# anerisheth19/CNN-MobileNet-V1-implementation-on-AWS-FPGA-using-OpenCL

Hardware: AMD Instinct MI355X
Metric: images/sec MobileNet-V1 1.0x224 fp32, batch 256; per-stage HBM GB/s vs roofline (higher is better)
Workload: dtype f32

## Files before the change

cnn-mobilenet-v1-implementation-on-aws-fpga-using-opencl_amd/csrc/mbn_abi.hip:

```cpp
#include "mbn_internal.h"

#include <initializer_list>
#include <new>

mbn_tunables g_mbn_tune;

namespace {

struct Span { const void *p; double bytes; const char *what; };

int span_check(mbn_context *ctx, const Span *sp, int n)
{
    std::lock_guard<std::mutex> lk(ctx->mu);
    if (ctx->allocs.empty()) return MBN_OK;
    for (int i = 0; i < n; i++) {
        if (!sp[i].p || sp[i].bytes <= 0) continue;
        const uintptr_t a = (uintptr_t)sp[i].p;
        auto it = ctx->allocs.upper_bound(a);
        if (it == ctx->allocs.begin()) continue;
        --it;
        if (a >= it->first + it->second) continue;
        const double room = (double)(it->first + it->second - a);
        if (sp[i].bytes > room) {
            snprintf(ctx->last_error, sizeof(ctx->last_error), "%s: call touches %.0f bytes, %.0f left in its %zu-byte mbn_alloc buffer",
// ... 729 lines not shown
                int channels, int classes, void *workspace, size_t workspace_bytes, void *stream)
{
    if (!ctx || !logits || !in || !fc_w || !workspace || batch <= 0 || rows <= 0 || cols <= 0 || channels <= 0 || classes <= 0) return MBN_EINVAL;
    if (batch > 4 || channels < 64 || channels > 1024 || (channels % 64) != 0) return MBN_EUNSUPPORTED;
    if (workspace_bytes < mbn_pool_fc_ws_bytes(channels, classes)) return MBN_EINVAL;
    hipStream_t s = stream ? (hipStream_t)stream : ctx->stream;
    MBN_SPANS(ctx, { in, 4.0 * batch * rows * cols * channels, "pool_fc input" }, { logits, 4.0 * batch * classes, "pool_fc logits" },
              { fc_w, 4.0 * classes * channels, "pool_fc filter" }, { workspace, (double)mbn_pool_fc_ws_bytes(channels, classes), "pool_fc workspace" });
    Scope sc(ctx, s);
    return sc.finish(mbn_launch_f32_pool_fc(ctx, s, (float *)logits, (const float *)in, (const float *)fc_w, (const float *)fc_bias, workspace,
                                            batch, rows * cols, channels, classes, 0, nullptr, nullptr, nullptr));
}

int mbn_classifier_tail_fused(mbn_context *ctx, void *topk_idx_i32, void *topk_prob_f32, void *probs, void *logits, const void *in, const void *fc_w,
                              const void *fc_bias, int batch, int rows, int cols, int channels, int classes, int k, void *workspace,
                              size_t workspace_bytes, void *stream)
{
    if (!ctx || !topk_idx_i32 || !topk_prob_f32 || !logits || !in || !fc_w || !workspace || batch <= 0 || rows <= 0 || cols <= 0 || channels <= 0 ||
        classes <= 0 || k < 1 || k > 8)
        return MBN_EINVAL;
    if (batch > 4 || channels < 64 || channels > 1024 || (channels % 64) != 0 || classes > 1024) return MBN_EUNSUPPORTED;
    if (workspace_bytes < mbn_pool_fc_ws_bytes(channels, classes)) return MBN_EINVAL;
    hipStream_t s = stream ? (hipStream_t)stream : ctx->stream;
    MBN_SPANS(ctx, { in, 4.0 * batch * rows * cols * channels, "classifier_tail_fused input" }, { logits, 4.0 * batch * classes, "classifier_tail_fused logits" },
              { fc_w, 4.0 * classes * channels, "classifier_tail_fused filter" }, { workspace, (double)mbn_pool_fc_ws_bytes(channels, classes), "classifier_tail_fused workspace" },
              { probs, 4.0 * batch * classes, "classifier_tail_fused probs" }, { topk_idx_i32, 4.0 * batch * k, "classifier_tail_fused idx" },
              { topk_prob_f32, 4.0 * batch * k, "classifier_tail_fused prob" });
    Scope sc(ctx, s);
    return sc.finish(mbn_launch_f32_pool_fc(ctx, s, (float *)logits, (const float *)in, (const float *)fc_w, (const float *)fc_bias, workspace,
                                            batch, rows * cols, channels, classes, k, (float *)probs, (int32_t *)topk_idx_i32, (float *)topk_prob_f32));
}

static int stem_fused_impl(mbn_context *ctx, void *out, const void *image, const void *w1, const void *s1, const void *b1,
                           const void *wd, const void *s2, const void *b2, const void *wp, const void *s3, const void *b3,
                           int batch, int res, int c1, int c3, void *stream, int in_u8, int bf16)
{
    if (!ctx || !out || !image) return MBN_EINVAL;
    hipStream_t s = stream ? (hipStream_t)stream : ctx->stream;
    if (mbn_stem_envelope(batch, res, c1, c3) != MBN_OK) return MBN_EUNSUPPORTED;
    MBN_SPANS(ctx, { image, (in_u8 ? 1.0 : 4.0) * batch * res * res * 3, "stem image" },
              { out, (bf16 ? 2.0 : 4.0) * batch * (res / 2) * (res / 2) * c3, "stem output" });
    if (check_ptrs({ w1, s1, b1, wd, s2, b2, wp, s3, b3 }) != MBN_OK) return MBN_EUNSUPPORTED;
    if (((uintptr_t)out % 16) != 0 || ((uintptr_t)image % (in_u8 ? 2 : 8)) != 0) return MBN_EINVAL;
    Scope sc(ctx, s);
    return sc.finish(mbn_launch_f32_stem(ctx, s, (float *)out, (const float *)image, (const float *)w1, (const float *)s1,
                                         (const float *)b1, (const float *)wd, (const float *)s2, (const float *)b2,
                                         (const float *)wp, (const float *)s3, (const float *)b3, batch, res, c1, c3, in_u8, bf16));
}

int mbn_stem_fused(mbn_context *ctx, void *out, const void *image, const void *w1, const void *s1, const void *b1,
                   const void *wd, const void *s2, const void *b2, const void *wp, const void *s3, const void *b3,
                   int batch, int res, int c1, int c3, void *stream)
{
    return stem_fused_impl(ctx, out, image, w1, s1, b1, wd, s2, b2, wp, s3, b3, batch, res, c1, c3, stream, 0, 0);
}

int mbn_stem_fused_u8(mbn_context *ctx, void *out, const void *image_u8, const void *w1, const void *s1, const void *b1,
                      const void *wd, const void *s2, const void *b2, const void *wp, const void *s3, const void *b3,
                      int batch, int res, int c1, int c3, void *stream)
{
    return stem_fused_impl(ctx, out, image_u8, w1, s1, b1, wd, s2, b2, wp, s3, b3, batch, res, c1, c3, stream, 1, 0);
}

int mbn_stem_fused_ex(mbn_context *ctx, void *out, const void *image, const void *w1, const void *s1, const void *b1,
                      const void *wd, const void *s2, const void *b2, const void *wp, const void *s3, const void *b3,
                      int batch, int res, int c1, int c3, int flags, void *stream)
{
    if (flags & ~(MBN_STEM_IN_U8 | MBN_STEM_BF16)) return MBN_EINVAL;
    return stem_fused_impl(ctx, out, image, w1, s1, b1, wd, s2, b2, wp, s3, b3, batch, res, c1, c3, stream,
                           (flags & MBN_STEM_IN_U8) != 0, (flags & MBN_STEM_BF16) != 0);
}

int mbn_dwpw_fused(mbn_context *ctx, void *out, const void *in, const void *wd, const void *s2, const void *b2,
                   const void *wp, const void *s3, const void *b3, int batch, int in_rows, int in_cols, int out_rows,
                   int out_cols, int cin, int cout, int stride, int pad_top, int pad_left, void *stream)
{
    if (!ctx) return MBN_EINVAL;
    hipStream_t s = stream ? (hipStream_t)stream : ctx->stream;
    const mbn_block_shape sh = { batch, in_rows, in_cols, out_rows, out_cols, cin, cout, stride, pad_top, pad_left };
    const mbn_block_params p = { wd, s2, b2, wp, s3, b3 };
    int rc = check_ptrs({ in, wd, s2, b2, wp, s3, b3, out });
    if (rc == MBN_OK) rc = mbn_block_envelope(&sh, MBN_DT_F32);
    if (rc != MBN_OK) return rc;
    MBN_SPANS(ctx, { in, 4.0 * batch * in_rows * in_cols * cin, "dwpw input" },
              { out, 4.0 * batch * out_rows * out_cols * cout, "dwpw output" }, { wd, 36.0 * cin, "dwpw depthwise filter" },
              { wp, 4.0 * cin * cout, "dwpw pointwise filter" });
    Scope sc(ctx, s);
    if (g_mbn_tune.pw_emul != 0 && g_mbn_tune.dwpw_variant == 0 && mbn_launch_f32_dwpw2_x6(ctx, s, sh, out, in, p) == MBN_OK)
        return sc.finish(MBN_OK);
    const int dv = g_mbn_tune.dwpw_variant;
    if ((dv == 11 || dv >= 300 || (dv == 0 && MBN_DWPW3_DEFAULT(stride, cin))) && mbn_f32_dwpw3_eligible(ctx, sh))
        return sc.finish(mbn_launch_f32_dwpw3(ctx, s, sh, out, in, p));
    const long tiles256 = (((long)batch * out_rows * out_cols + 127) / 128) * (cout / 256);
    const bool small = tiles256 < ctx->num_cus;
    if (dv != 1 && (dv >= 2 || (cout % 256) != 0 || small || stride == 2))
        return sc.finish(mbn_launch_f32_dwpw2(ctx, s, sh, out, in, p));
    return sc.finish(mbn_launch_f32_dwpw(ctx, s, sh, out, in, p));
}

int mbn_blocks_resident_bf16(mbn_context *ctx, void *out, const void *in, const mbn_block_params *blocks, int nblocks, int batch,
                             int rows, int cols, int channels, void *stream)
{
    if (!ctx || !out || !in || !blocks || batch <= 0) return MBN_EINVAL;
    const mbn_block_shape sh = { batch, rows, cols, rows, cols, channels, channels, 1, 1, 1 };
    if (mbn_resident_envelope(&sh, nblocks) != MBN_OK) return MBN_EUNSUPPORTED;
    hipStream_t s = stream ? (hipStream_t)stream : ctx->stream;
    const double act = 2.0 * batch * rows * cols * channels;
    MBN_SPANS(ctx, { in, act, "resident blocks input" }, { out, act, "resident blocks output" });
    for (int i = 0; i < nblocks; i++) {
        if (!blocks[i].wd || !blocks[i].s2 || !blocks[i].b2 || !blocks[i].wp_bf16 || !blocks[i].s3 || !blocks[i].b3) return MBN_EINVAL;
        MBN_SPANS(ctx, { blocks[i].wd, 36.0 * channels, "resident blocks depthwise filter" }, { blocks[i].wp_bf16, 2.0 * channels * channels, "resident blocks pointwise filter" },
                  { blocks[i].s2, 4.0 * channels, "resident blocks scale" }, { blocks[i].b3, 4.0 * channels, "resident blocks shift" });
    }
    int rc = check_ptrs({ out, in });
    for (int i = 0; i < nblocks && rc == MBN_OK; i++) rc = check_ptrs(blocks[i]);
    if (rc != MBN_OK) return rc;
    Scope sc(ctx, s);
    return sc.finish(mbn_launch_bf16_res_blocks(ctx, s, out, in, blocks, nblocks, batch, rows, cols));
}

int mbn_tail_resident_bf16(mbn_context *ctx, void *out, const void *in, const mbn_block_params *blocks, int batch, int rows, int cols, int c0, int c1,
                           void *stream)
{
    if (!ctx || !out || !in || !blocks || batch <= 0) return MBN_EINVAL;
    const mbn_block_shape b0 = { batch, rows, cols, rows / 2, cols / 2, c0, c1, 2, 0, 0 };
    const mbn_block_shape b1 = { batch, rows / 2, cols / 2, rows / 2, cols / 2, c1, c1, 1, 1, 1 };
    if (mbn_tail_envelope(&b0, &b1) != MBN_OK) return MBN_EUNSUPPORTED;
    hipStream_t s = stream ? (hipStream_t)stream : ctx->stream;
    MBN_SPANS(ctx, { in, 2.0 * batch * rows * cols * c0, "resident tail input" }, { out, 2.0 * batch * c1, "resident tail output" });
    for (int i = 0; i < 2; i++) {
        if (!blocks[i].wd || !blocks[i].s2 || !blocks[i].b2 || !blocks[i].wp_bf16 || !blocks[i].s3 || !blocks[i].b3) return MBN_EINVAL;
        const int ci = i ? c1 : c0;
        MBN_SPANS(ctx, { blocks[i].wd, 36.0 * ci, "resident tail depthwise filter" }, { blocks[i].wp_bf16, 2.0 * ci * c1, "resident tail pointwise filter" },
                  { blocks[i].s2, 4.0 * ci, "resident tail scale" }, { blocks[i].b2, 4.0 * ci, "resident tail shift" },
                  { blocks[i].s3, 4.0 * c1, "resident tail scale" }, { blocks[i].b3, 4.0 * c1, "resident tail shift" });
    }
    int rc = ((uintptr_t)out % 2) ? MBN_EUNSUPPORTED : check_ptrs({ in });
    for (int i = 0; i < 2 && rc == MBN_OK; i++) rc = check_ptrs(blocks[i]);
    if (rc != MBN_OK) return rc;
    Scope sc(ctx, s);
    return sc.finish(mbn_launch_bf16_tail(ctx, s, out, in, blocks, batch, rows, cols));
}

int mbn_dwpw_fused_bf16(mbn_context *ctx, void *out, const void *in, const void *wd, const void *s2, const void *b2,
                        const void *wp_bf16, const void *s3, const void *b3, int batch, int in_rows, int in_cols, int out_rows,
                        int out_cols, int cin, int cout, int stride, int pad_top, int pad_left, void *stream)
{
    if (!ctx) return MBN_EINVAL;
    hipStream_t s = stream ? (hipStream_t)stream : ctx->stream;
    const mbn_block_shape sh = { batch, in_rows, in_cols, out_rows, out_cols, cin, cout, stride, pad_top, pad_left };
    const mbn_block_params p = { wd, s2, b2, wp_bf16, s3, b3 };
    int rc = check_ptrs({ in, wd, s2, b2, wp_bf16, s3, b3, out });
    if (rc == MBN_OK) rc = mbn_block_envelope(&sh, MBN_DT_BF16);
    if (rc != MBN_OK) return rc;
    MBN_SPANS(ctx, { in, 2.0 * batch * in_rows * in_cols * cin, "dwpw input" },
              { out, 2.0 * batch * out_rows * out_cols * cout, "dwpw output" }, { wd, 36.0 * cin, "dwpw depthwise filter" },
              { wp_bf16, 2.0 * cin * cout, "dwpw pointwise filter" });
    Scope sc(ctx, s);
#ifdef MBN_LAB
    if (g_mbn_tune.dwpw_variant == 1 && (cout % 128) == 0 && (cin % 64) == 0)
        return sc.finish(mbn_launch_bf16_dwpw(ctx, s, sh, out, in, p));
#endif
    return sc.finish(mbn_launch_bf16_dwpw2(ctx, s, sh, out, in, p));
}

int mbn_convert_f32_to_bf16(mbn_context *ctx, void *dst_bf16, const void *src_f32, size_t count, void *stream)
{
    if (!ctx || !dst_bf16 || !src_f32) return MBN_EINVAL;
    if (count == 0) return MBN_OK;
    hipStream_t s = stream ? (hipStream_t)stream : ctx->stream;
    MBN_SPANS(ctx, { src_f32, 4.0 * count, "convert source" }, { dst_bf16, 2.0 * count, "convert destination" });
    Scope sc(ctx, s);
    return sc.finish(mbn_launch_convert(ctx, s, dst_bf16, src_f32, count, 1));
// ... 47 lines not shown
```

cnn-mobilenet-v1-implementation-on-aws-fpga-using-opencl_amd/csrc/mbn_f32_pw.hip:

```cpp
#include "mbn_internal.h"
#include "mbn_epilogue.h"

namespace {

typedef float f4 __attribute__((ext_vector_type(4)));
typedef mbn_f16v f16v;
typedef __bf16 bf8 __attribute__((ext_vector_type(8)));

#ifdef MBN_LAB
__device__ unsigned long long g_pw_clk[8][4];
#endif

__device__ unsigned long long g_pw_clk_acc[9][2];

struct PwArgs {
    void *out;
    const void *in, *filt;
    const float *scale, *shift;
    long m;
    int k, n, act;
    int mt, nt;
    int out_f32;
    int fast_epi;
    int loop2;
// ... 373 lines not shown
                }
            }
        }
        __builtin_amdgcn_sched_barrier(0);
        if (!more) break;
        vb = nvb;
    }
#ifdef MBN_LAB
    if (clk) { g_pw_clk[blockIdx.x][1] = __builtin_amdgcn_s_memtime(); g_pw_clk[blockIdx.x][3] = __builtin_amdgcn_s_memrealtime(); }
#endif
    if (hclk) {
        atomicAdd(&g_pw_clk_acc[blockIdx.x][0], __builtin_amdgcn_s_memtime() - hc0);
        atomicAdd(&g_pw_clk_acc[blockIdx.x][1], __builtin_amdgcn_s_memrealtime() - hr0);
        if (blockIdx.x == 0) atomicAdd(&g_pw_clk_acc[8][0], 1ull);
    }
}

template <typename T>
__global__ __launch_bounds__(256) void pw_generic(PwArgs a)
{
    const long t = (long)blockIdx.x * blockDim.x + threadIdx.x;
    if (t >= a.m * a.n) return;
    const long row = t / a.n;
    const int col = (int)(t % a.n);
    const T *ip = reinterpret_cast<const T *>(a.in) + row * a.k, *fp = reinterpret_cast<const T *>(a.filt) + (long)col * a.k;
    float acc = 0.f;
    for (int i = 0; i < a.k; i++) acc = fmaf((float)ip[i], (float)fp[i], acc);
    float v = fmaf(acc, a.scale ? a.scale[col] : 1.f, a.shift ? a.shift[col] : 0.f);
    if (a.act == MBN_ACT_RELU6) v = fminf(fmaxf(v, 0.f), 6.f);
    else if (a.act == MBN_ACT_RELU) v = fmaxf(v, 0.f);
    if (sizeof(T) == 4 || a.out_f32) reinterpret_cast<float *>(a.out)[t] = v;
    else reinterpret_cast<__bf16 *>(a.out)[t] = (__bf16)v;
}

template <typename T, int BM, int BN, int WM, int WN>
void launch_cfg(PwArgs &a, hipStream_t s, int num_cus)
{
    constexpr int NT = 64 * (BM / WM) * (BN / WN);
    constexpr int BKE = 8 * (16 / (int)sizeof(T));
    a.mt = (int)((a.m + BM - 1) / BM);
    a.nt = (a.n + BN - 1) / BN;
    const int nbuf = a.k <= BKE ? 1 : 2;
    const int lds_bytes = nbuf * (BM + BN) * BKB + (nbuf == 2 ? 2 * SSMAX * 4 : 0);
    int per_cu = 160 * 1024 / lds_bytes;
    const int wave_cap = 32 / (NT / 64);
    if (per_cu > wave_cap) per_cu = wave_cap;
    if (per_cu > 4) per_cu = 4;
    if (g_mbn_tune.misc > 0) per_cu = g_mbn_tune.misc;
    const long nwg = (long)a.mt * a.nt;
    long grid_l = (long)num_cus * per_cu;
    if (grid_l > nwg || g_mbn_tune.misc >= 1000 || nbuf == 1) grid_l = nwg;
    a.xn = 1;
    {
        const double filt_bytes = (double)a.n * a.k * sizeof(T);
        int xn = filt_bytes >= 16.0 * 1048576 ? 4 : filt_bytes >= 4.0 * 1048576 ? 2 : 1;
        if (g_mbn_tune.pw_xn > 0) xn = g_mbn_tune.pw_xn;
        if ((xn == 2 || xn == 4) && grid_l < nwg && (grid_l % 8) == 0 && a.nt >= xn && a.mt >= 8 / xn) a.xn = xn;
    }
    const dim3 grid((unsigned)grid_l), block(NT);
    const bool kfull = (a.k % BKE) == 0;
    const bool glds = kfull && nbuf == 2 && g_mbn_tune.pw_stage != 1;
    if (nbuf == 1) {
        if (kfull) hipLaunchKernelGGL((pw_gemm<T, BM, BN, WM, WN, 1, true, false>), grid, block, 0, s, a);
        else hipLaunchKernelGGL((pw_gemm<T, BM, BN, WM, WN, 1, false, false>), grid, block, 0, s, a);
    } else {
#ifdef MBN_LAB
        if (glds && sizeof(T) == 4 && g_mbn_tune.exp1 > 0 && ((BM == 64 && BN == 64) || (BM == 128 && BN == 128))) {
            switch (g_mbn_tune.exp1) {
#define MBN_ABL_CASE(v) case v: hipLaunchKernelGGL((pw_gemm<T, BM, BN, WM, WN, 2, true, true, v>), grid, block, 0, s, a); return;
            MBN_ABL_CASE(1) MBN_ABL_CASE(2) MBN_ABL_CASE(3) MBN_ABL_CASE(4) MBN_ABL_CASE(7) MBN_ABL_CASE(8) MBN_ABL_CASE(9) MBN_ABL_CASE(10) MBN_ABL_CASE(12) MBN_ABL_CASE(15)
#undef MBN_ABL_CASE
            default: break;
            }
        }
#endif
        if (glds) hipLaunchKernelGGL((pw_gemm<T, BM, BN, WM, WN, 2, true, true>), grid, block, 0, s, a);
#ifdef MBN_LAB
        else if (kfull) hipLaunchKernelGGL((pw_gemm<T, BM, BN, WM, WN, 2, true, false>), grid, block, 0, s, a);
#endif
        else hipLaunchKernelGGL((pw_gemm<T, BM, BN, WM, WN, 2, false, false>), grid, block, 0, s, a);
    }
}

}

int mbn_launch_f32_pointwise(const mbn_call &c, void *out, const void *in, const void *filt, long m, int cin,
                             int op_size)
{
    const bool bf = c.dtype == MBN_DT_BF16;
    PwArgs a;
    a.out = out; a.in = in; a.filt = filt; a.scale = c.scale; a.shift = c.shift;
    a.m = m; a.k = cin; a.n = op_size; a.act = c.act; a.mt = a.nt = 0;
    a.out_f32 = bf && (c.io_flags & MBN_IO_OUT_F32) ? 1 : 0;
    a.loop2 = (g_mbn_tune.conv_variant == 8 || ((cin / (bf ? 64 : 32)) & 1) || (cin % (bf ? 64 : 32)) ||
               (double)m * cin * (bf ? 2 : 4) >= 4294967296.0 || (double)op_size * cin * (bf ? 2 : 4) >= 4294967296.0) ? 0 : 1;
    a.no_ss = g_mbn_tune.conv_variant == 7 ? 1 : 0;
    a.no_cw = g_mbn_tune.exp0 == 77 ? 1 : 0;
    a.clk = g_mbn_tune.pw_clock.load(std::memory_order_relaxed) ? 1 : 0;
    a.fast_epi = (g_mbn_tune.conv_variant == 9 || (double)m * op_size * 4.0 >= 4294967296.0) ? 0 : 1;
    if (m <= 0 || (long)((m + 31) / 32) * ((op_size + 31) / 32) > 0x7fffffffL) return MBN_EINVAL;
    const int epc = bf ? 8 : 4;
    const bool fast = (cin % epc) == 0 && ((uintptr_t)in % 16) == 0 && ((uintptr_t)filt % 16) == 0;
    if (!fast) {
        long total = m * op_size;
        dim3 grid((unsigned)((total + 255) / 256));
        if (bf) hipLaunchKernelGGL(pw_generic<__bf16>, grid, dim3(256), 0, c.stream, a);
        else hipLaunchKernelGGL(pw_generic<float>, grid, dim3(256), 0, c.stream, a);
        return MBN_OK;
    }
    const int ring_mode = g_mbn_tune.pw_ring;
    if (!bf && g_mbn_tune.pw_emul != 0 && mbn_launch_f32_pw_emul(c, (float *)out, (const float *)in, (const float *)filt, m, cin, op_size) == MBN_OK)
        return MBN_OK;
    if (!bf && g_mbn_tune.pw_tile == 0 && mbn_launch_f32_pw_splitk(c, (float *)out, (const float *)in, (const float *)filt, m, cin, op_size) == MBN_OK)
        return MBN_OK;
#ifdef MBN_LAB
    if (bf && (c.io_flags & MBN_IO_FILT_PACKED) && ring_mode == 6 && g_mbn_tune.pw_tile == 0 &&
        mbn_launch_bf16_pw_wide(c, out, in, (const char *)filt + mbn_packed_filter_offset(op_size, cin), m, cin, op_size) == MBN_OK)
        return MBN_OK;
#endif
#ifdef MBN_LAB
    if (bf && ring_mode == 7 && g_mbn_tune.pw_tile == 0) {
        long done = 0;
        if (mbn_launch_bf16_pw_big(c, out, in, filt, m, cin, op_size, &done) == MBN_OK) {
            if (done < m && g_mbn_tune.exp2 < 98)
                return mbn_launch_f32_pointwise(c, (char *)out + done * op_size * 2, (const char *)in + done * cin * 2, filt, m - done, cin, op_size);
            return MBN_OK;
        }
    }
#endif
#ifdef MBN_LAB
    if (bf && ring_mode == 8 && g_mbn_tune.pw_tile == 0 && mbn_launch_bf16_pw_rf(c, out, in, filt, m, cin, op_size) == MBN_OK)
        return MBN_OK;
#endif
    if (bf && (ring_mode == 0 || ring_mode == 5 || ring_mode == 8) && cin >= 256 && g_mbn_tune.pw_tile == 0 && mbn_launch_bf16_pw_stream(c, out, in, filt, m, cin, op_size, true) == MBN_OK)
        return MBN_OK;
    if (bf && (ring_mode == 4 || ((ring_mode == 0 || ring_mode == 6) && (cin <= 128 || (cin <= 256 && op_size <= 256)))) && g_mbn_tune.pw_tile == 0 &&
        mbn_launch_bf16_pw_stream(c, out, in, filt, m, cin, op_size) == MBN_OK)
        return MBN_OK;
#ifdef MBN_LAB
    if (bf && ring_mode >= 2 && (ring_mode == 2 || cin == 64) && g_mbn_tune.pw_tile == 0 &&
        mbn_launch_bf16_pw_ring(c, out, in, filt, m, cin, op_size) == MBN_OK)
        return MBN_OK;
#endif
    if (!bf && (g_mbn_tune.pw_tile == 9 || (g_mbn_tune.pw_tile == 0 && MBN_PW3_DEFAULT(m, cin, op_size, c.ctx->num_cus))) &&
        mbn_launch_f32_pw3(c, (float *)out, (const float *)in, (const float *)filt, m, cin, op_size) == MBN_OK)
        return MBN_OK;
    int tile = g_mbn_tune.pw_tile;
    if (tile == 9 || tile == 10) tile = 0;
    if (!MBN_LAB_BUILD && tile != 2 && tile != 3 && tile != 5) tile = 0;
    if (tile == 0) {
        const long big_tiles = ((m + 127) / 128) * ((op_size + 63) / 64);
        if (big_tiles < 2L * c.ctx->num_cus || op_size <= 64 || m <= 16384) tile = 3;
        else if (!bf && (cin >= 512 || (cin >= 256 && op_size >= 512))) tile = 3;
        else if ((bf || cin <= 256) && op_size >= 128) tile = 5;
        else tile = 2;
    }
    const int cus = c.ctx->num_cus;
    if (bf) {
        switch (tile) {
        case 3:
            if (op_size >= 128) launch_cfg<__bf16, 64, 128, 32, 64>(a, c.stream, cus);
            else launch_cfg<__bf16, 64, 64, 32, 32>(a, c.stream, cus);
            break;
        case 5: launch_cfg<__bf16, 128, 128, 32, 64>(a, c.stream, cus); break;
        case 2: launch_cfg<__bf16, 128, 64, 64, 32>(a, c.stream, cus); break;
#ifdef MBN_LAB
// ... 57 lines not shown
```

cnn-mobilenet-v1-implementation-on-aws-fpga-using-opencl_amd/csrc/mbn_internal.h:

```cpp
#pragma once
#include <hip/hip_runtime.h>
#include <stdint.h>
#include <stdio.h>
#include <string.h>

#include <atomic>
#include <map>
#include <mutex>
#include <vector>

#include "mbn.h"
#include "mbn_envelope.h"

struct mbn_emul_img {
    void *p = nullptr;
    size_t bytes = 0;
    size_t src_bytes = 0;
    bool built = false;
};

struct mbn_context {
    int device = 0;
    hipStream_t stream = nullptr;
    hipEvent_t ev_start = nullptr, ev_stop = nullptr;
// ... 59 lines not shown
};
extern mbn_tunables g_mbn_tune;

struct mbn_call {
    mbn_context *ctx;
    hipStream_t stream;
    int batch;
    int act;
    int pad_top, pad_left;
    int in_rows, in_cols;
    int cin;
    int g0, g1;
    uint32_t quirks;
    const float *scale, *shift;
    int dtype;
    int io_flags;
};

int mbn_launch_lit_convolute(const mbn_call &c, uint8_t *out, const uint8_t *r, const uint8_t *g, const uint8_t *b,
                             const int32_t *filt, int rows, int cols, int fs, int stride, int op_size);
int mbn_launch_lit_depthwise(const mbn_call &c, uint8_t *out, const uint8_t *in, const int32_t *filt, int rows,
                             int cols, int fs, int stride, int op_size);
int mbn_launch_lit_pointwise(const mbn_call &c, uint8_t *out, const uint8_t *in, const int32_t *filt, int rows,
                             int cols, int cin, int op_size);
int mbn_launch_lit_pool(const mbn_call &c, uint8_t *out, const uint8_t *in, int rows, int cols, int fs, int op_size);

int mbn_launch_f32_conv(const mbn_call &c, void *out, const void *in, const float *filt, int rows, int cols, int fs,
                        int stride, int op_size);
int mbn_launch_f32_depthwise(const mbn_call &c, void *out, const void *in, const float *filt, int rows, int cols,
                             int fs, int stride, int channels);
int mbn_launch_f32_pointwise(const mbn_call &c, void *out, const void *in, const void *filt, long m, int cin,
                             int op_size);
int mbn_launch_f32_pw_splitk(const mbn_call &c, float *out, const float *in, const float *filt, long m, int cin, int op_size);
int mbn_launch_f32_pw_emul(const mbn_call &c, float *out, const float *in, const float *filt, long m, int cin, int op_size);
int mbn_pw_emul_filter_image(mbn_context *ctx, hipStream_t stream, const float *filt, int n, int k, int bn, int paired,
                             const unsigned **img, unsigned *bytes);
void mbn_pw_emul_invalidate(mbn_context *ctx, const void *dst, size_t bytes);
int mbn_launch_bf16_pw_ring(const mbn_call &c, void *out, const void *in, const void *filt, long m, int cin, int op_size);
int mbn_launch_bf16_pw_wide(const mbn_call &c, void *out, const void *in, const void *fpk, long m, int cin, int op_size);
int mbn_launch_pack_filter_bf16(mbn_context *ctx, hipStream_t s, void *dst, const void *src, int n, int k);
int mbn_bf16_pw_wide_eligible(long m, int cin, int op_size);
int mbn_launch_bf16_pw_rf(const mbn_call &c, void *out, const void *in, const void *filt, long m, int cin, int op_size);
int mbn_launch_bf16_pw_stream(const mbn_call &c, void *out, const void *in, const void *filt, long m, int cin, int op_size, bool m16 = false);
int mbn_launch_bf16_pw_big(const mbn_call &c, void *out, const void *in, const void *filt, long m, int cin, int op_size, long *rows_done);
int mbn_launch_f32_pool(const mbn_call &c, void *out, const void *in, int rows, int cols, int fs, int channels);
size_t mbn_pool_fc_ws_bytes(int channels, int classes);
int mbn_launch_f32_pool_fc(mbn_context *ctx, hipStream_t s, float *out, const float *in, const float *w, const float *bias, void *ws,
                           int batch, int pix, int channels, int classes, int k, float *probs, int32_t *topk_idx, float *topk_prob);
static inline void mbn_udiv_magic(unsigned d, unsigned *m, unsigned *s)
{
    if (d <= 1) { *m = 0; *s = 0; return; }
    unsigned l = 0;
    while ((1u << l) < d) l++;
    const unsigned long long p = 1ull << (31 + l);
    *m = (unsigned)((p + d - 1) / d);
    *s = l - 1;
}

int mbn_launch_f32_dwpw(mbn_context *ctx, hipStream_t stream, const mbn_block_shape &s, void *out, const void *in, const mbn_block_params &p);
int mbn_launch_f32_dwpw2(mbn_context *ctx, hipStream_t stream, const mbn_block_shape &s, void *out, const void *in, const mbn_block_params &p);
int mbn_launch_f32_dwpw2_x6(mbn_context *ctx, hipStream_t stream, const mbn_block_shape &s, void *out, const void *in, const mbn_block_params &p);
int mbn_launch_bf16_dwpw(mbn_context *ctx, hipStream_t stream, const mbn_block_shape &s, void *out, const void *in, const mbn_block_params &p);
int mbn_launch_bf16_dwpw2(mbn_context *ctx, hipStream_t stream, const mbn_block_shape &s, void *out, const void *in, const mbn_block_params &p);
template <typename Args>
static inline void mbn_block_args(Args &a, const mbn_block_shape &s, void *out, const void *in, const mbn_block_params &p, double esize)
{
    a.out = (decltype(a.out))out; a.in = (decltype(a.in))in;
    a.wd = (const float *)p.wd; a.s2 = (const float *)p.s2; a.b2 = (const float *)p.b2; a.s3 = (const float *)p.s3; a.b3 = (const float *)p.b3;
    a.m = (long)s.batch * s.out_rows * s.out_cols;
    a.h = s.in_rows; a.w = s.in_cols; a.ho = s.out_rows; a.wo = s.out_cols;
    a.cin = s.cin; a.cout = s.cout; a.pad_top = s.pad_top; a.pad_left = s.pad_left;
    mbn_udiv_magic((unsigned)s.out_cols, &a.wo_m, &a.wo_s);
    mbn_udiv_magic((unsigned)s.out_rows, &a.ho_m, &a.ho_s);
    a.in_bytes = (unsigned)(esize * s.batch * s.in_rows * s.in_cols * s.cin);
}
#define MBN_PW3_DEFAULT(m, cin, n, cus) ((cin) <= 256 && (n) <= 256 && (m) >= 128L * (cus))
int mbn_launch_f32_pw3(const mbn_call &c, float *out, const float *in, const float *filt, long m, int cin, int op_size);
int mbn_launch_bf16_tail(mbn_context *ctx, hipStream_t stream, void *out, const void *in, const mbn_block_params *blocks, int batch, int rows, int cols);
int mbn_launch_bf16_res_blocks(mbn_context *ctx, hipStream_t stream, void *out, const void *in, const mbn_block_params *blocks, int nblocks, int batch,
                               int rows, int cols);
#define MBN_DWPW3_DEFAULT(stride, cin) ((stride) == 1 && (cin) >= 128)
int mbn_f32_dwpw3_eligible(const mbn_context *ctx, const mbn_block_shape &s);
int mbn_launch_f32_dwpw3(mbn_context *ctx, hipStream_t stream, const mbn_block_shape &s, void *out, const void *in, const mbn_block_params &p);
int mbn_launch_f32_stem(mbn_context *ctx, hipStream_t stream, float *out, const float *in, const float *w1,
                        const float *s1, const float *b1, const float *wd, const float *s2, const float *b2,
                        const float *wp, const float *s3, const float *b3, int batch, int res, int c1, int c3, int in_u8, int bf16);
int mbn_launch_convert(mbn_context *ctx, hipStream_t s, void *dst, const void *src, size_t count, int to_bf16);
int mbn_launch_f32_softmax(mbn_context *ctx, hipStream_t s, float *probs, int32_t *argmax, const float *logits,
                           int batch, int classes);
int mbn_launch_f32_softmax_topk(mbn_context *ctx, hipStream_t s, float *probs, int32_t *topk_idx, float *topk_prob,
                                const float *logits, int batch, int classes, int k);
int mbn_launch_normalize(mbn_context *ctx, hipStream_t s, float *out, const uint8_t *in, size_t count, float scale,
                         float bias);

static inline int mbn_same_pad(int in, int out, int k, int stride)
{
    int total = (out - 1) * stride + k - in;
    if (total < 0) total = 0;
    return total / 2;
}
```

cnn-mobilenet-v1-implementation-on-aws-fpga-using-opencl_amd/host/mbn_envelope.c:

```c
#include "mbn_envelope.h"
#include "mbn.h"

int mbn_block_envelope(const mbn_block_shape *s, int dtype)
{
    const int bf = dtype == MBN_DT_BF16;
    if (!bf && dtype != MBN_DT_F32) return MBN_EUNSUPPORTED;
    if (s->batch <= 0 || (s->stride != 1 && s->stride != 2) || s->cin > MBN_CMAX || s->cout > MBN_COUT_MAX || (s->out_cols & 1) ||
        s->out_rows <= 0 || s->out_cols <= 0 || s->in_rows <= 0 || s->in_cols <= 0 || s->pad_top < 0 || s->pad_left < 0)
        return MBN_EUNSUPPORTED;
    if (bf ? (s->cin != 32 && (s->cin < 64 || (s->cin % 64) != 0)) || s->cout < 64 || (s->cout % 64) != 0
           : s->cin < 32 || (s->cin % 32) != 0 || s->cout < 128 || (s->cout % 128) != 0)
        return MBN_EUNSUPPORTED;
    const double es = bf ? 2.0 : 4.0;
    if (es * s->batch * s->in_rows * s->in_cols * s->cin >= (double)MBN_OOB) return MBN_EUNSUPPORTED;
    if ((long)s->batch * s->out_rows * s->out_cols > 0x7fffff00L) return MBN_EUNSUPPORTED;
    if (es * ((double)s->batch * s->out_rows * s->out_cols + 256.0) * s->cout >= 4294967296.0) return MBN_EUNSUPPORTED;
    return MBN_OK;
}

int mbn_resident_envelope(const mbn_block_shape *s, int nblocks)
{
    if (s->cin != 256 || s->cout != 256 || s->stride != 1 || s->pad_top != 1 || s->pad_left != 1 || s->in_rows < 1 || s->in_cols < 1 ||
        s->out_rows != s->in_rows || s->out_cols != s->in_cols || nblocks < 1 || nblocks > MBN_RES_MAXBLK)
        return MBN_EUNSUPPORTED;
    if (s->in_rows * s->in_cols > MBN_RES_YROWS || (s->in_rows + 2) * (s->in_cols + 2) > MBN_RES_XPIX) return MBN_EUNSUPPORTED;
    return MBN_OK;
}

int mbn_tail_envelope(const mbn_block_shape *b0, const mbn_block_shape *b1)
{
    const int h = b0->in_rows, w = b0->in_cols;
    if (b0->cin != 256 || b0->cout != 512 || h < 2 || w < 2 || h > MBN_TAIL_MAXSIDE || w > MBN_TAIL_MAXSIDE || (h & 1) || (w & 1))
        return MBN_EUNSUPPORTED;
    if (b0->stride != 2 || b0->pad_top != 0 || b0->pad_left != 0 || b0->out_rows != h / 2 || b0->out_cols != w / 2) return MBN_EUNSUPPORTED;
    if (b1->batch != b0->batch || b1->cin != b0->cout || b1->cout != b0->cout || b1->stride != 1 || b1->pad_top != 1 || b1->pad_left != 1 ||
        b1->in_rows != b0->out_rows || b1->in_cols != b0->out_cols || b1->out_rows != b1->in_rows || b1->out_cols != b1->in_cols)
        return MBN_EUNSUPPORTED;
    if (2.0 * b0->batch * h * w * b0->cin >= 4294967296.0) return MBN_EUNSUPPORTED;
    return MBN_OK;
}

int mbn_stem_envelope(int batch, int res, int c1, int c3)
{
    if (!((c1 == 32 && c3 == 64) || (c1 == 16 && c3 == 32)) || res < 32 || (res % 32) != 0 || batch <= 0) return MBN_EUNSUPPORTED;
    if ((long)batch * (res / 2 / MBN_STEM_TH) * (res / 2 / MBN_STEM_TW) >= 0x7fffffffL) return MBN_EUNSUPPORTED;
    return MBN_OK;
}
```

cnn-mobilenet-v1-implementation-on-aws-fpga-using-opencl_amd/host/mbn_envelope.h:

```cpp
#pragma once

#ifdef __cplusplus
extern "C" {
#endif

#define MBN_CMAX 1024
#define MBN_COUT_MAX 1024
#define MBN_OOB 0xF0000000u
#define MBN_RES_XPIX 144
#define MBN_RES_YROWS 104
#define MBN_RES_MAXBLK 8
#define MBN_TAIL_MAXSIDE 10
#define MBN_STEM_TH 8
#define MBN_STEM_TW 16

typedef struct mbn_block_shape {
    int batch, in_rows, in_cols, out_rows, out_cols, cin, cout, stride, pad_top, pad_left;
} mbn_block_shape;

int mbn_block_envelope(const mbn_block_shape *s, int dtype);
int mbn_resident_envelope(const mbn_block_shape *s, int nblocks);
int mbn_tail_envelope(const mbn_block_shape *b0, const mbn_block_shape *b1);
int mbn_stem_envelope(int batch, int res, int c1, int c3);

#ifdef __cplusplus
}
#endif
```

Before: 91970.

## Add fused depthwise-into-GEMM dwpw4 kernel for wide stride-1 f32 blocks

```diff
diff --git a/cnn-mobilenet-v1-implementation-on-aws-fpga-using-opencl_amd/csrc/mbn_abi.hip b/cnn-mobilenet-v1-implementation-on-aws-fpga-using-opencl_amd/csrc/mbn_abi.hip
--- a/cnn-mobilenet-v1-implementation-on-aws-fpga-using-opencl_amd/csrc/mbn_abi.hip
+++ b/cnn-mobilenet-v1-implementation-on-aws-fpga-using-opencl_amd/csrc/mbn_abi.hip
@@ -835,13 +835,16 @@
     int rc = check_ptrs({ in, wd, s2, b2, wp, s3, b3, out });
     if (rc == MBN_OK) rc = mbn_block_envelope(&sh, MBN_DT_F32);
     if (rc != MBN_OK) return rc;
+    const int dv = g_mbn_tune.dwpw_variant;
+    const bool gemm_form = mbn_block_gemm_envelope(&sh) == MBN_OK && g_mbn_tune.pw_emul == 0 && dv == 0;
+    if (!gemm_form && (out_cols & 1)) return MBN_EUNSUPPORTED;
     MBN_SPANS(ctx, { in, 4.0 * batch * in_rows * in_cols * cin, "dwpw input" },
               { out, 4.0 * batch * out_rows * out_cols * cout, "dwpw output" }, { wd, 36.0 * cin, "dwpw depthwise filter" },
               { wp, 4.0 * cin * cout, "dwpw pointwise filter" });
     Scope sc(ctx, s);
+    if (gemm_form) return sc.finish(mbn_launch_f32_dwpw4(ctx, s, sh, out, in, p));
     if (g_mbn_tune.pw_emul != 0 && g_mbn_tune.dwpw_variant == 0 && mbn_launch_f32_dwpw2_x6(ctx, s, sh, out, in, p) == MBN_OK)
         return sc.finish(MBN_OK);
-    const int dv = g_mbn_tune.dwpw_variant;
     if ((dv == 11 || dv >= 300 || (dv == 0 && MBN_DWPW3_DEFAULT(stride, cin))) && mbn_f32_dwpw3_eligible(ctx, sh))
         return sc.finish(mbn_launch_f32_dwpw3(ctx, s, sh, out, in, p));
     const long tiles256 = (((long)batch * out_rows * out_cols + 127) / 128) * (cout / 256);
diff --git a/cnn-mobilenet-v1-implementation-on-aws-fpga-using-opencl_amd/csrc/mbn_f32_pw.hip b/cnn-mobilenet-v1-implementation-on-aws-fpga-using-opencl_amd/csrc/mbn_f32_pw.hip
--- a/cnn-mobilenet-v1-implementation-on-aws-fpga-using-opencl_amd/csrc/mbn_f32_pw.hip
+++ b/cnn-mobilenet-v1-implementation-on-aws-fpga-using-opencl_amd/csrc/mbn_f32_pw.hip
@@ -479,6 +479,224 @@
     }
 }
 
+struct Dwpw4Args {
+    float *out;
+    const float *in, *wd, *s2, *b2, *wp, *s3, *b3;
+    long m;
+    int h, w, ho, wo, cin, cout, pad_top, pad_left;
+    unsigned in_bytes;
+    int mt, nt, xn;
+};
+
+template <int BM, int BN, int WM, int WN>
+__global__ __launch_bounds__(64 * (BM / WM) * (BN / WN)) void dwpw4_f32(Dwpw4Args a)
+{
+    constexpr int WAVES_N = BN / WN;
+    constexpr int NT = 64 * (BM / WM) * WAVES_N;
+    constexpr int MI = WM / 32, NI = WN / 32;
+    constexpr int BKE = 32;
+    constexpr int B_LD = BN * 8 / NT;
+    static_assert(BM * 8 == NT && B_LD * NT == BN * 8, "one A chunk per thread");
+    __shared__ __attribute__((aligned(16))) float lds[2 * (BM + BN) * BKF + 2 * SSMAX];
+    float *const sc_s = lds + 2 * (BM + BN) * BKF, *const sh_s = sc_s + SSMAX;
+    for (int i = threadIdx.x; i < a.cout; i += NT) { sc_s[i] = a.s3[i]; sh_s[i] = a.b3[i]; }
+    __syncthreads();
+
+    const int nwg = a.mt * a.nt;
+    const int tid = threadIdx.x, lane = tid & 63, wave = tid >> 6;
+    const int wm = (wave / WAVES_N) * WM, wn = (wave % WAVES_N) * WN;
+    const int li = lane & 31, lh = lane >> 5;
+    const int nk = a.cin / BKE;
+    const int st_ch = tid & 7, st_row = tid >> 3;
+    int st_rowb[B_LD];
+#pragma unroll
+    for (int p = 0; p < B_LD; p++) st_rowb[p] = (p * NT + tid) >> 3;
+    int fr_a[4], fr_b[4];
+#pragma unroll
+    for (int g = 0; g < 4; g++) {
+        fr_a[g] = swz(wm + li, 2 * g + lh);
+        fr_b[g] = swz(wn + li, 2 * g + lh);
+    }
+    const int wave_u = __builtin_amdgcn_readfirstlane(wave);
+    const int wm_u = (wave_u / WAVES_N) * WM, wn_u = (wave_u % WAVES_N) * WN;
+    const __amdgpu_buffer_rsrc_t orsrc = mbn_make_rsrc(a.out, (unsigned)(a.m * a.cout * 4));
+    const __amdgpu_buffer_rsrc_t irs = mbn_make_rsrc(a.in, a.in_bytes);
+    const __amdgpu_buffer_rsrc_t wrs = mbn_make_rsrc(a.wd, 36u * a.cin), srs = mbn_make_rsrc(a.s2, 4u * a.cin),
+                                 brs = mbn_make_rsrc(a.b2, 4u * a.cin);
+    const unsigned b_bytes = (unsigned)a.cout * a.cin * 4u, cin4 = 4u * a.cin;
+
+    unsigned tap[9], b_vo[B_LD];
+    f4 xt[9], wt[9], ws, wb;
+    const int xm = 8 / a.xn;
+    auto set_tile = [&](int vb, long &m0, int &n0) {
+        int mtile, ntile;
+        if (a.xn > 1) {
+            const int x = vb & 7, j = vb >> 3, gm = x / a.xn, gn = x % a.xn;
+            const int mlo = (int)((long)a.mt * gm / xm), nlo = a.nt * gn / a.xn, nn = a.nt * (gn + 1) / a.xn - nlo;
+            mtile = mlo + j / nn;
+            ntile = nlo + j % nn;
+        } else {
+            const int lid = xcd_remap(vb, nwg);
+            mtile = lid / a.nt;
+            ntile = lid % a.nt;
+        }
+        n0 = ntile * BN;
+        m0 = (long)mtile * BM;
+        long gm = m0 + st_row;
+        if (gm >= a.m) gm = a.m - 1;
+        const unsigned px = (unsigned)gm, hw = (unsigned)a.ho * (unsigned)a.wo;
+        const unsigned img = px / hw, r = px - img * hw, oy = r / (unsigned)a.wo, ox = r - oy * (unsigned)a.wo;
+#pragma unroll
+        for (int dy = 0; dy < 3; dy++)
+#pragma unroll
+            for (int dx = 0; dx < 3; dx++) {
+                const int iy = (int)oy - a.pad_top + dy, ix = (int)ox - a.pad_left + dx;
+                tap[3 * dy + dx] = ((unsigned)iy < (unsigned)a.h && (unsigned)ix < (unsigned)a.w)
+                                       ? (((img * a.h + iy) * a.w + ix) * (unsigned)a.cin + st_ch * 4) * 4u : MBN_OOB;
+            }
+#pragma unroll
+        for (int p = 0; p < B_LD; p++)
+            b_vo[p] = ((unsigned)(n0 + st_rowb[p]) * (unsigned)a.cin + ((st_ch ^ (st_rowb[p] >> 1)) & 7) * 4) * 4u;
+    };
+    auto stage = [&](int kt, int buf) __attribute__((always_inline)) {
+        const int kb = kt * BKB;
+#pragma unroll
+        for (int j = 0; j < 9; j++) xt[j] = __builtin_bit_cast(f4, __builtin_amdgcn_raw_buffer_load_b128(irs, tap[j], kb, 0));
+#pragma unroll
+        for (int j = 0; j < 9; j++) wt[j] = __builtin_bit_cast(f4, __builtin_amdgcn_raw_buffer_load_b128(wrs, st_ch * 16u, kb + j * cin4, 0));
+        ws = __builtin_bit_cast(f4, __builtin_amdgcn_raw_buffer_load_b128(srs, st_ch * 16u, kb, 0));
+        wb = __builtin_bit_cast(f4, __builtin_amdgcn_raw_buffer_load_b128(brs, st_ch * 16u, kb, 0));
+        __builtin_amdgcn_sched_barrier(0);
+        lds_dma_rows(a.wp, b_bytes, lds + buf * (BM + BN) * BKF + BM * BKF, b_vo, kb, wave_u, B_LD, NT);
+    };
+    auto dw_store = [&](int buf) __attribute__((always_inline)) {
+        f4 acc = f4{ 0.f, 0.f, 0.f, 0.f };
+#pragma unroll
+        for (int j = 0; j < 9; j++)
+            acc = f4{ fmaf(xt[j].x, wt[j].x, acc.x), fmaf(xt[j].y, wt[j].y, acc.y), fmaf(xt[j].z, wt[j].z, acc.z), fmaf(xt[j].w, wt[j].w, acc.w) };
+        acc = f4{ fminf(fmaxf(fmaf(acc.x, ws.x, wb.x), 0.f), 6.f), fminf(fmaxf(fmaf(acc.y, ws.y, wb.y), 0.f), 6.f),
+                  fminf(fmaxf(fmaf(acc.z, ws.z, wb.z), 0.f), 6.f), fminf(fmaxf(fmaf(acc.w, ws.w, wb.w), 0.f), 6.f) };
+        *reinterpret_cast<f4 *>(lds + buf * (BM + BN) * BKF + swz(st_row, st_ch)) = acc;
+    };
+
+    constexpr int NSTF = 16 * MI * NI;
+    bool prev_fast = false;
+    long m0;
+    int n0;
+    int vb = blockIdx.x;
+    int vb_end = nwg;
+    if (a.xn > 1) {
+        const int x = vb & 7, gm = x / a.xn, gn = x % a.xn;
+        const int cnt = (int)((long)a.mt * (gm + 1) / xm - (long)a.mt * gm / xm) * (a.nt * (gn + 1) / a.xn - a.nt * gn / a.xn);
+        vb_end = (cnt << 3) + x;
+    }
+    if (vb >= vb_end) return;
+    set_tile(vb, m0, n0);
+    stage(0, 0);
+    dw_store(0);
+
+    for (;;) {
+        f16v acc[MI][NI];
+#pragma unroll
+        for (int mi = 0; mi < MI; mi++)
+#pragma unroll
+            for (int ni = 0; ni < NI; ni++)
+#pragma unroll
+                for (int r = 0; r < 16; r++) acc[mi][ni][r] = 0.f;
+        if (prev_fast) asm volatile("s_waitcnt vmcnt(%0) lgkmcnt(0)\n\ts_barrier" ::"n"(NSTF) : "memory");
+        else __syncthreads();
+        f4 fa[2][MI], fb[2][NI];
+        auto ldfrag = [&](const float *base, int g, int slot) __attribute__((always_inline)) {
+#pragma unroll
+            for (int mi = 0; mi < MI; mi++) fa[slot][mi] = *reinterpret_cast<const f4 *>(base + fr_a[g] + mi * 32 * BKF);
+#pragma unroll
+            for (int ni = 0; ni < NI; ni++) fb[slot][ni] = *reinterpret_cast<const f4 *>(base + BM * BKF + fr_b[g] + ni * 32 * BKF);
+        };
+        auto mfma_group = [&](int slot) __attribute__((always_inline)) {
+#pragma unroll
+            for (int s = 0; s < 4; s++)
+#pragma unroll
+                for (int mi = 0; mi < MI; mi++)
+#pragma unroll
+                    for (int ni = 0; ni < NI; ni++)
+                        acc[mi][ni] = __builtin_amdgcn_mfma_f32_32x32x2f32(fa[slot][mi][s], fb[slot][ni][s], acc[mi][ni], 0, 0, 0);
+        };
+        auto ktile_head = [&](const int CUR, const bool NEXT, int kt) __attribute__((always_inline)) {
+            const float *base = lds + CUR * (BM + BN) * BKF;
+            if (NEXT) stage(kt + 1, CUR ^ 1);
+#pragma unroll
+            for (int g = 0; g < 3; g++) {
+                ldfrag(base, g + 1, (g + 1) & 1);
+                __builtin_amdgcn_sched_barrier(0);
+                mfma_group(g & 1);
+                __builtin_amdgcn_sched_barrier(0);
+            }
+            if (NEXT) dw_store(CUR ^ 1);
+        };
+        auto ktile_tail = [&](const int CUR, const bool NEXT) __attribute__((always_inline)) {
+            if (NEXT) ldfrag(lds + (CUR ^ 1) * (BM + BN) * BKF, 0, 0);
+            __builtin_amdgcn_sched_barrier(0);
+            mfma_group(1);
+            __builtin_amdgcn_sched_barrier(0);
+        };
+        ldfrag(lds, 0, 0);
+        int kt = 0;
+        for (; kt + 2 < nk; kt += 2) {
+            ktile_head(0, true, kt);
+            __syncthreads();
+            ktile_tail(0, true);
+            ktile_head(1, true, kt + 1);
+            __syncthreads();
+            ktile_tail(1, true);
+        }
+        ktile_head(0, true, kt);
+        __syncthreads();
+        ktile_tail(0, true);
+        ktile_head(1, false, kt + 1);
+        __syncthreads();
+        ktile_tail(1, false);
+
+        const long cm0 = m0;
+        const int cn0 = n0;
+        const int nvb = vb + gridDim.x;
+        const bool more = nvb < vb_end;
+        if (more) {
+            set_tile(nvb, m0, n0);
+            stage(0, 0);
+        }
+        __builtin_amdgcn_sched_barrier(0);
+        prev_fast = cm0 + BM <= a.m;
+        if (prev_fast) mbn_store_relu6_f32<MI, NI, 0, float>(orsrc, (unsigned)a.cout, (unsigned)cm0 + wm_u, cn0 + wn_u, lane, acc, sc_s, sh_s, (unsigned)a.m, a.cout);
+        else mbn_store_relu6_f32<MI, NI, 1, float>(orsrc, (unsigned)a.cout, (unsigned)cm0 + wm_u, cn0 + wn_u, lane, acc, sc_s, sh_s, (unsigned)a.m, a.cout);
+        __builtin_amdgcn_sched_barrier(0);
+        if (!more) break;
+        dw_store(0);
+        vb = nvb;
+    }
+}
+
+}
+
+int mbn_launch_f32_dwpw4(mbn_context *ctx, hipStream_t stream, const mbn_block_shape &s, void *out, const void *in, const mbn_block_params &p)
+{
+    constexpr int BM = 32, BN = 256;
+    Dwpw4Args a;
+    a.out = (float *)out; a.in = (const float *)in;
+    a.wd = (const float *)p.wd; a.s2 = (const float *)p.s2; a.b2 = (const float *)p.b2;
+    a.wp = (const float *)p.wp_bf16; a.s3 = (const float *)p.s3; a.b3 = (const float *)p.b3;
+    a.m = (long)s.batch * s.out_rows * s.out_cols;
+    a.h = s.in_rows; a.w = s.in_cols; a.ho = s.out_rows; a.wo = s.out_cols;
+    a.cin = s.cin; a.cout = s.cout; a.pad_top = s.pad_top; a.pad_left = s.pad_left;
+    a.in_bytes = (unsigned)(4.0 * s.batch * s.in_rows * s.in_cols * s.cin);
+    a.mt = (int)((a.m + BM - 1) / BM);
+    a.nt = s.cout / BN;
+    const long nwg = (long)a.mt * a.nt;
+    long grid = 2L * ctx->num_cus;
+    if (grid > nwg) grid = nwg;
+    const int xn = 4.0 * s.cout * s.cin >= 4.0 * 1048576 ? 2 : 1;
+    a.xn = (xn == 2 && grid < nwg && (grid % 8) == 0 && a.nt >= xn && a.mt >= 8 / xn) ? xn : 1;
+    hipLaunchKernelGGL((dwpw4_f32<BM, BN, 32, 64>), dim3((unsigned)grid), dim3(256), 0, stream, a);
+    return MBN_OK;
 }
 
 int mbn_launch_f32_pointwise(const mbn_call &c, void *out, const void *in, const void *filt, long m, int cin,
diff --git a/cnn-mobilenet-v1-implementation-on-aws-fpga-using-opencl_amd/csrc/mbn_internal.h b/cnn-mobilenet-v1-implementation-on-aws-fpga-using-opencl_amd/csrc/mbn_internal.h
--- a/cnn-mobilenet-v1-implementation-on-aws-fpga-using-opencl_amd/csrc/mbn_internal.h
+++ b/cnn-mobilenet-v1-implementation-on-aws-fpga-using-opencl_amd/csrc/mbn_internal.h
@@ -165,6 +165,7 @@
 #define MBN_DWPW3_DEFAULT(stride, cin) ((stride) == 1 && (cin) >= 128)
 int mbn_f32_dwpw3_eligible(const mbn_context *ctx, const mbn_block_shape &s);
 int mbn_launch_f32_dwpw3(mbn_context *ctx, hipStream_t stream, const mbn_block_shape &s, void *out, const void *in, const mbn_block_params &p);
+int mbn_launch_f32_dwpw4(mbn_context *ctx, hipStream_t stream, const mbn_block_shape &s, void *out, const void *in, const mbn_block_params &p);
 int mbn_launch_f32_stem(mbn_context *ctx, hipStream_t stream, float *out, const float *in, const float *w1,
                         const float *s1, const float *b1, const float *wd, const float *s2, const float *b2,
                         const float *wp, const float *s3, const float *b3, int batch, int res, int c1, int c3, int in_u8, int bf16);
diff --git a/cnn-mobilenet-v1-implementation-on-aws-fpga-using-opencl_amd/host/mbn_envelope.c b/cnn-mobilenet-v1-implementation-on-aws-fpga-using-opencl_amd/host/mbn_envelope.c
--- a/cnn-mobilenet-v1-implementation-on-aws-fpga-using-opencl_amd/host/mbn_envelope.c
+++ b/cnn-mobilenet-v1-implementation-on-aws-fpga-using-opencl_amd/host/mbn_envelope.c
@@ -1,10 +1,22 @@
 #include "mbn_envelope.h"
 #include "mbn.h"
+
+int mbn_block_gemm_envelope(const mbn_block_shape *s)
+{
+    if (s->batch <= 0 || s->stride != 1 || s->cin != s->cout || s->cin < 512 || (s->cin % 256) != 0 || s->cout > MBN_COUT_MAX ||
+        s->out_rows <= 0 || s->out_cols <= 0 || s->in_rows <= 0 || s->in_cols <= 0 || s->pad_top < 0 || s->pad_left < 0)
+        return MBN_EUNSUPPORTED;
+    if (4.0 * s->batch * s->in_rows * s->in_cols * s->cin >= (double)MBN_OOB) return MBN_EUNSUPPORTED;
+    if ((long)s->batch * s->out_rows * s->out_cols > 0x7fffff00L) return MBN_EUNSUPPORTED;
+    if (4.0 * ((double)s->batch * s->out_rows * s->out_cols + 256.0) * s->cout >= 4294967296.0) return MBN_EUNSUPPORTED;
+    return MBN_OK;
+}
 
 int mbn_block_envelope(const mbn_block_shape *s, int dtype)
 {
     const int bf = dtype == MBN_DT_BF16;
     if (!bf && dtype != MBN_DT_F32) return MBN_EUNSUPPORTED;
+    if (!bf && mbn_block_gemm_envelope(s) == MBN_OK) return MBN_OK;
     if (s->batch <= 0 || (s->stride != 1 && s->stride != 2) || s->cin > MBN_CMAX || s->cout > MBN_COUT_MAX || (s->out_cols & 1) ||
         s->out_rows <= 0 || s->out_cols <= 0 || s->in_rows <= 0 || s->in_cols <= 0 || s->pad_top < 0 || s->pad_left < 0)
         return MBN_EUNSUPPORTED;
diff --git a/cnn-mobilenet-v1-implementation-on-aws-fpga-using-opencl_amd/host/mbn_envelope.h b/cnn-mobilenet-v1-implementation-on-aws-fpga-using-opencl_amd/host/mbn_envelope.h
--- a/cnn-mobilenet-v1-implementation-on-aws-fpga-using-opencl_amd/host/mbn_envelope.h
+++ b/cnn-mobilenet-v1-implementation-on-aws-fpga-using-opencl_amd/host/mbn_envelope.h
@@ -19,6 +19,7 @@
 } mbn_block_shape;
 
 int mbn_block_envelope(const mbn_block_shape *s, int dtype);
+int mbn_block_gemm_envelope(const mbn_block_shape *s);
 int mbn_resident_envelope(const mbn_block_shape *s, int nblocks);
 int mbn_tail_envelope(const mbn_block_shape *b0, const mbn_block_shape *b1);
 int mbn_stem_envelope(int batch, int res, int c1, int c3);
```

Result: no change. 92020 (median of 6 runs) (+0.1%).
